# lunarring/latentblending

Hardware: AMD Instinct MI355X
Metric: transition frames/sec, SDXL-Turbo 512x512 4-step 15-branch (higher is better)
Workload: dtype f16; 1 GPU; SDXL-Turbo 512x512, num_inference_steps=4, nmb_max_branches=15 (17 frames/transition), fp16, fixed_seeds=[420,421], anchors not recycled; frontier_width=16, hipgraphs=True, parallelism=single GPU

## Files before the change

### include/lb_hip.h

```cpp
#ifndef LB_HIP_H
#define LB_HIP_H

#include <stdint.h>

#ifdef __cplusplus
extern "C" {
#endif

typedef uint16_t lb_half;

int lb_version(void);
const char* lb_last_error_string(void);
int lb_device_info(int device, int* cu_count, long* lds_per_cu, char* arch, int arch_len);

int lb_slerp_pairs_f16(const void* const* p0, const void* const* p1, void* const* out,
                       const double* fracts, int npairs, long n, void* stream);
int lb_slerp_pairs_f32(const void* const* p0, const void* const* p1, void* const* out,
                       const double* fracts, int npairs, long n, void* stream);
int lb_slerp_pairs_f64(const void* const* p0, const void* const* p1, void* const* out,
                       const double* fracts, int npairs, long n, void* stream);
int lb_slerp_batched_f16(const void* p0, const void* p1, void* out, const double* fracts_dev,
                         long npairs, long n, void* stream);
int lb_slerp_strided_f16(const void* p0, long stride0, const void* p1, long stride1, void* out,
                         const double* fracts_dev, long npairs, long n, void* stream);
// ... 12 lines not shown

enum {
    LB_GEMM_OUT_F32 = 1,
    LB_GEMM_RES_F32 = 2,
    LB_GEMM_GEGLU = 4,
    LB_GEMM_TRANS_OUT = 8,
    LB_GEMM_SILU = 16,
    LB_GEMM_RELU = 32,
    LB_GEMM_QUICK_GELU = 128,
    LB_GEMM_GELU = 256,
    LB_GEMM_CH_STATS = 512,
    LB_GEMM_HALO_RAGGED = 1024,
    LB_GEMM_HALO_KSPLIT = 4096,
    LB_GEMM_C64 = 2048,
    LB_GEMM_GN_A = 8192,
    LB_GEMM_LN_A = 64
};

typedef struct LbGemmParams {
    const lb_half* A;
    const lb_half* W;
    void* C;
    const float* bias;
    const void* residual;
    const lb_half* rowvec;
    float* partial;
    int M, N, K;
    int lda, ldw, ldc, ldr, ld_rowvec, rows_per_batch;
    float alpha;
    int flags;
// ... 14 lines not shown
} LbGemmParams;

int lb_gemm_f16(const LbGemmParams* params, void* stream);
long lb_gemm_workspace_bytes(int M, int N);
void lb_gemm_set_tuning(int tile, int splitk);
void lb_gemm_set_pp_auto(int on);
void lb_gemm_pp_set_group(int gm);
void lb_gemm_set_depth(int depth);
int lb_gemm_plan(const LbGemmParams* p, int* tile, int* splitk, long* blocks);
int lb_conv3x3_halo_f16(const LbGemmParams* params, void* stream);
int lb_conv3x3_narrow_f16(const LbGemmParams* params, void* stream);
void lb_conv_halo_set_persistent(int on);
void lb_conv_halo_plan(const LbGemmParams* params, int* kind, int* tile_w, long* items, long* grid);
#include "lb_hip_ksplit.h"
#include "lb_hip_gn_a.h"
int lb_gemm_ch_stat_rows(const LbGemmParams* params);
int lb_upconv2x_halo_f16(const LbGemmParams* params, void* stream);
void lb_gemm_set_halo(int mode);
void lb_gemm_set_wide_store(int on);
void lb_gemm_set_t192_waves8(int on);
void lb_gemm_set_kgroups(int on);
void lb_gemm_set_lean_epilogue(int on);
void lb_gemm_set_variant(int variant, int stages);

void lb_groupnorm_set_l3_chunk(long bytes);
int lb_groupnorm_from_stats(const void* x, void* y, const float* gamma, const float* beta, const float* ch_stats,
                            void* workspace, int B, int HW, int C, int ldx, int ldy, int groups, float eps, int silu,
                            int x_is_f32, int stat_rows_per_sample, void* stream);
long lb_groupnorm_workspace_bytes(int B, int groups);
int lb_groupnorm_nhwc(const void* x, void* y, const float* gamma, const float* beta, void* workspace,
// ... 81 lines not shown
```

### latentblending_amd/csrc/conv3_narrow.hip

```cpp
#include "lb_common.h"
#include "lb_gemm.h"

typedef __attribute__((address_space(1))) const void* gptr_t;
typedef __attribute__((address_space(3))) void* lptr_t;

#define NARROW_T 16
#define NARROW_HW (NARROW_T + 2)
#define NARROW_HR (NARROW_HW * NARROW_HW)
#define NARROW_HRG ((NARROW_HR + 7) / 8)
#define NARROW_LDS (NARROW_HRG * 8 * 64)

template <bool GNA>
__global__ void __launch_bounds__(256, 2) conv3x3_narrow_kernel(const LbGemmParams p) {
    __shared__ __attribute__((aligned(16))) f16 halo[NARROW_LDS];
    const int tid = threadIdx.x, lane = tid & 63, wave = tid >> 6;
    const int g = lane >> 4, l16 = lane & 15;
    const int tiles_x = p.Win / NARROW_T, tiles_y = p.Hin / NARROW_T;
    int tile = blockIdx.x;
    const int x0 = (tile % tiles_x) * NARROW_T;
    tile /= tiles_x;
    const int y0 = (tile % tiles_y) * NARROW_T;
    const int b = tile / tiles_y;
    const lb_half* zero = reinterpret_cast<const lb_half*>(p.zero_page);
    const int nchunks = p.Cin / 64;
// ... 84 lines not shown
            float o[4];
#pragma unroll
            for (int r = 0; r < 4; ++r) o[r] = acc[i][r] * p.alpha + bias[r];
            if (p.flags & LB_GEMM_OUT_F32)
                *reinterpret_cast<f32x4*>((float*)p.C + m * p.ldc + n) = (f32x4){o[0], o[1], o[2], o[3]};
            else
                *reinterpret_cast<f16x4*>((f16*)p.C + m * p.ldc + n) = (f16x4){(f16)o[0], (f16)o[1], (f16)o[2], (f16)o[3]};
        }
    }
}

int lb_conv3x3_narrow_eligible(const LbGemmParams& p) {
    if (!p.conv || p.KH != 3 || p.KW != 3 || p.stride != 1 || p.pad != 1 || p.ups || p.scatter) return 0;
    if (p.Hout != p.Hin || p.Wout != p.Win || p.Cin % 64 != 0 || p.K != 9 * p.Cin) return 0;
    if (p.N > 16 || p.N % 4 != 0 || p.zero_page == nullptr) return 0;
    if (p.flags & ~(LB_GEMM_OUT_F32 | LB_GEMM_HALO_KSPLIT | LB_GEMM_GN_A)) return 0;
    if (p.residual != nullptr || p.rowvec != nullptr) return 0;
    if (p.Win % NARROW_T != 0 || p.Hin % NARROW_T != 0 || p.M % (p.Hin * p.Win) != 0) return 0;
    if ((long)p.M * p.ldx >= (1l << 34)) return 0;
    return 1;
}

static long narrow_tiles(const LbGemmParams& p) {
    return (long)(p.M / (p.Hin * p.Win)) * (p.Hin / NARROW_T) * (p.Win / NARROW_T);
}

int lb_conv3x3_narrow_check(const LbGemmParams& p) {
    LB_REQUIRE(narrow_tiles(p) < (1l << 31), "conv3x3 narrow: too many tiles for one launch");
    LB_REQUIRE(!(p.flags & LB_GEMM_GN_A) || (p.gn_table != nullptr && (reinterpret_cast<uintptr_t>(p.gn_table) & 15) == 0),
               "conv3x3 narrow: LB_GEMM_GN_A needs gn_table = the 16-byte aligned [B][Cin] float2 table of lb_groupnorm_affine_from_stats");
    return 0;
// ... 21 lines not shown
```

### latentblending_amd/csrc/gemm.hip

```cpp
#include "lb_common.h"
#include "lb_gemm.h"

#define BK 64

template <int N> struct Int { static constexpr int value = N; };

template <int BM, int BN, bool CONV, bool GEGLU, int D>
__global__ void __launch_bounds__(256) gemm_f16_kernel(const LbGemmParams p) {
    constexpr int AI = BM * 8 / 256;
    constexpr int WI = BN * 8 / 256;
    constexpr int TM = BM / 32;
    constexpr int TN = BN / 32;
    __shared__ __attribute__((aligned(16))) f16 lds[2 * (BM + BN) * BK];
    f16* const As = lds;
    f16* const Ws = lds + 2 * BM * BK;

    const int tid = threadIdx.x;
    const int lane = tid & 63, wave = tid >> 6;
    const int wave_m = wave >> 1, wave_n = wave & 1;
    const int g = lane >> 4, l16 = lane & 15;

    const int n_blocks = GEGLU ? (p.N / 2 + BN / 2 - 1) / (BN / 2) : (p.N + BN - 1) / BN;
    int bid = blockIdx.x;
    {
// ... 263 lines not shown
int lb_upconv_halo_launch(LbGemmParams p, hipStream_t stream);
int lb_conv3_c64_check(const LbGemmParams& p);
int lb_conv3_c64_launch(LbGemmParams p, hipStream_t stream);
void lb_conv3_c64_grid(const LbGemmParams& p, long& items, long& grid);
#define LB_HALO_MIN_BLOCKS 96
static int g_halo = 1;
extern "C" void lb_gemm_set_halo(int mode) { g_halo = mode; }
static bool use_halo(const LbGemmParams& p) {
    if (g_halo == 0 || g_force_tile || !lb_conv3x3_halo_eligible(p)) return false;
    return g_halo == 2 || lb_conv3x3_halo_blocks(p) >= LB_HALO_MIN_BLOCKS;
}

int lb_gemm_pp_eligible(const LbGemmParams& p);
int lb_gemm_launch_pp(const LbGemmParams& p, dim3 grid, hipStream_t stream);
int lb_gemm_launch_glds(const LbGemmParams& p, int tile, int stages, dim3 grid, hipStream_t stream);
void lb_gemm_glds_init();
static int g_variant = 1, g_stages = 0;
extern "C" void lb_gemm_set_variant(int variant, int stages) {
    g_variant = variant < 0 ? 1 : variant;
    g_stages = variant < 0 ? 0 : stages;
    if (variant == 1) lb_gemm_glds_init();
}

int g_lb_wide_store = 1;
extern "C" void lb_gemm_set_wide_store(int on) { g_lb_wide_store = on; }
int g_lb_lean_epilogue = 1;
extern "C" void lb_gemm_set_lean_epilogue(int on) { g_lb_lean_epilogue = on; }

extern "C" long lb_gemm_workspace_bytes(int M, int N) {
    return (long)16 * M * N * (long)sizeof(float);
}

template <int BM, int BN>
static void launch_depth(const LbGemmParams& p, int depth, dim3 grid, hipStream_t stream) {
    switch (depth) {
        case 1: launch_variant<BM, BN, 1>(p, grid, stream); break;
        case 2: launch_variant<BM, BN, 2>(p, grid, stream); break;
        case 3: launch_variant<BM, BN, 3>(p, grid, stream); break;
        default: launch_variant<BM, BN, 4>(p, grid, stream); break;
    }
}

static int default_depth(const LbGemmParams& p, int tile) {
    if (tile == 1) return p.conv ? 1 : 3;
    if (tile == 2) return 3;
    return 4;
}

static int gemm_launch_impl(LbGemmParams p, int tile, int depth, int variant, int stages, dim3 grid,
                            hipStream_t stream) {
    if (tile == 9) {
        lb_gemm_launch_pp(p, grid, stream);
    } else if (variant == 1 && p.zero_page != nullptr) {
        lb_gemm_launch_glds(p, tile, stages, grid, stream);
    } else {
        if (depth <= 0) depth = default_depth(p, tile);
        if (tile == 1) launch_depth<128, 128>(p, depth, grid, stream);
        else if (tile == 2) launch_depth<128, 64>(p, depth, grid, stream);
        else launch_depth<64, 64>(p, depth, grid, stream);
    }
    int rc = lb_check_launch("lb_gemm_f16");
    if (rc) return rc;
    if (p.splitk > 1) {
        const long quads = (long)p.M * (p.N / 4);
        long gsz = (quads + 255) / 256;
// ... 71 lines not shown
        if (splitk > k_tiles) splitk = k_tiles;
        if (splitk < 1) splitk = 1;
        if (tile == 9 && !g_force_splitk) splitk = 1;
        if (tile >= 4 && tile != 11 && !g_force_splitk) splitk = 1;
    }
    if (!g_force_tile && g_kgroups && tile == 3 && splitk == 1 && !p.conv && g_variant == 1 && p.zero_page != nullptr && nblk <= 200 &&
        (p.K + BK - 1) / BK >= 8)
        tile = 11;
    tile_out = tile;
    splitk_out = splitk;
    nblk_out = nblk;
}

extern "C" int lb_gemm_plan(const LbGemmParams* pp, int* tile, int* splitk, long* blocks) {
    LB_REQUIRE(pp != nullptr && pp->M > 0 && pp->N > 0 && pp->K > 0, "lb_gemm_plan: empty problem");
    int t = 0, sk = 1;
    long nb = 0;
    if (pp->flags & LB_GEMM_C64) {
        if (const int rc = lb_conv3_c64_check(*pp)) return rc;
        long items = 0;
        t = 12;
        lb_conv3_c64_grid(*pp, items, nb);
    }
    else if (g_halo != 0 && !g_force_tile && lb_conv3x3_narrow_eligible(*pp)) { t = 8; nb = (long)pp->M / 256; }
    else if (use_halo(*pp)) { t = 6; nb = lb_conv3x3_halo_blocks(*pp); }
    else if (pp->flags & LB_GEMM_HALO_KSPLIT) {
        LbGemmParams q = *pp;
        q.flags &= ~LB_GEMM_HALO_KSPLIT;
        q.partial = nullptr;
        gemm_plan(q, t, sk, nb);
// ... 30 lines not shown
            k = 8;
            f = lb_conv_halo_gn_a_mode() != 0;
        } else if (use_halo(p) && lb_conv3x3_halo_gn_a_able(p)) {
            k = 3;
            f = lb_conv3x3_halo_gn_a_policy(p);
        }
    }
    if (fuse) *fuse = f;
    if (kind) *kind = k;
}

extern "C" int lb_gemm_f16(const LbGemmParams* pp, void* stream) {
    LbGemmParams p = *pp;
    const bool geglu = (p.flags & LB_GEMM_GEGLU) != 0;
    LB_REQUIRE(p.M > 0 && p.N > 0 && p.K > 0, "lb_gemm_f16: empty problem");
    LB_REQUIRE(p.K % 8 == 0 && p.ldw % 8 == 0, "lb_gemm_f16: K and ldw must be multiples of 8");
    LB_REQUIRE(p.N % 4 == 0 && (geglu ? p.N % 8 == 0 : true), "lb_gemm_f16: N must be a multiple of 4");
    LB_REQUIRE(p.ldc % 4 == 0 || (p.flags & LB_GEMM_TRANS_OUT), "lb_gemm_f16: ldc must be a multiple of 4");
    if (p.conv) {
        LB_REQUIRE(p.Cin % 8 == 0 && p.ldx % 8 == 0, "lb_gemm_f16: conv Cin/ldx must be multiples of 8");
        LB_REQUIRE(p.K == p.KH * p.KW * p.Cin, "lb_gemm_f16: conv K != KH*KW*Cin");
        LB_REQUIRE(p.M % (p.Hout * p.Wout) == 0, "lb_gemm_f16: conv M must be B*Hout*Wout");
        if (p.scatter)
            LB_REQUIRE(p.KH == 2 && p.KW == 2 && p.stride == 1 && p.ups == 0 && p.Hout == p.Hin && p.Wout == p.Win &&
                           !(p.flags & (LB_GEMM_TRANS_OUT | LB_GEMM_GEGLU)) && p.residual == nullptr,
                       "lb_gemm_f16: sub-pixel conv needs KH=KW=2, stride 1, Hout=Hin, no residual");
    } else {
        LB_REQUIRE(p.lda % 8 == 0, "lb_gemm_f16: lda must be a multiple of 8");
    }
    if (p.flags & LB_GEMM_LN_A) {
// ... 21 lines not shown
        if (const int rc = lb_conv3x3_halo_check(p)) return rc;
        LB_DISPATCH("lb_conv3x3_halo_f16", lb_conv3x3_halo_launch(p, s));
    }
    LB_REQUIRE(!(p.flags & LB_GEMM_GN_A), "lb_gemm_f16: LB_GEMM_GN_A is implemented by the whole-tile 3x3 halo conv and the narrow-N conv only "
                                          "(ask lb_conv_halo_gn_a_plan before flagging a conv)");
    if (p.flags & LB_GEMM_HALO_KSPLIT) {
        p.flags &= ~LB_GEMM_HALO_KSPLIT;
        p.partial = nullptr;
    }
    LB_REQUIRE(!(p.flags & LB_GEMM_CH_STATS), "lb_gemm_f16: LB_GEMM_CH_STATS is implemented by the halo-tile conv kernels only "
                                              "(check lb_gemm_plan == 6 / lb_conv_halo_plan before asking for it)");
    int tile = 0, splitk = 1;
    long nblk = 0;
    gemm_plan(p, tile, splitk, nblk);
    p.splitk = splitk;
    const int depth = g_depth, variant = g_variant;
    int stages = g_stages;
    if (variant == 1) {
        lb_gemm_glds_init();
        if (stages == 0)
            stages = (tile == 3 || tile == 4 || tile == 7 || tile == 10 || tile == 11) ? 3 : 2;
    }
    const dim3 grid((unsigned)nblk, 1, (unsigned)splitk);
    LB_DISPATCH("lb_gemm_f16", gemm_launch_impl(p, tile, depth, variant, stages, grid, s));
}
```

### latentblending_amd/csrc/gemm_glds.hip

```cpp
#include <type_traits>
#include "lb_common.h"
#include "lb_gemm.h"

#define BK 64
#ifndef LB_GLDS_LEAN
#define LB_GLDS_LEAN 1
#endif
#ifndef LB_ABLATE
#define LB_ABLATE 0
#endif
#ifndef LB_BURST
#define LB_BURST 0
#endif
typedef __attribute__((address_space(1))) const void* gptr_t;
typedef __attribute__((address_space(3))) void* lptr_t;

template <int N> __device__ __forceinline__ void wait_vm_barrier() {
    asm volatile("s_waitcnt vmcnt(%0)\n\ts_barrier" ::"n"(N) : "memory");
}

typedef _Float16 lb_h2 __attribute__((ext_vector_type(2)));
template <int TM>
__device__ __forceinline__ void ln_accumulate(const f16x8 (&af)[TM], float (&sum)[TM], float (&sq)[TM]) {
    const lb_h2 one2 = {(f16)1.f, (f16)1.f};
#pragma unroll
    for (int i = 0; i < TM; ++i)
#pragma unroll
        for (int e = 0; e < 4; ++e) {
            const lb_h2 x = {af[i][2 * e], af[i][2 * e + 1]};
            sum[i] = __builtin_amdgcn_fdot2(x, one2, sum[i], false);
            sq[i] = __builtin_amdgcn_fdot2(x, x, sq[i], false);
        }
}

template <int BM, int BN, bool CONV, bool GEGLU, int S, int WMW, int LNA = 0, int KG = 1>
__global__ void __launch_bounds__(WMW * 128 * KG) gemm_f16_glds_kernel(const LbGemmParams p) {
    static_assert(KG == 1 || !CONV, "K-groups: plain / GEGLU GEMMs only");
    constexpr int NT = WMW * 128;
    constexpr int RPI = NT / 8;
    constexpr int AI = BM * 8 / NT;
    constexpr int WI = (BN * 8 + NT - 1) / NT;
    constexpr int NL = AI + WI;
    constexpr int WROWS = BM / WMW;
    constexpr int WPAD = WI * RPI;
    static_assert(BM * 8 % NT == 0, "A tile rows must be a whole number of staging rounds");
    constexpr int TM = WROWS / 16, TN = BN / 32;
    constexpr int STAGE = (BM + WPAD) * BK;
    extern __shared__ __attribute__((aligned(16))) f16 lds_all[];

    const int kgrp = KG > 1 ? __builtin_amdgcn_readfirstlane((int)threadIdx.x / NT) : 0;
    const int tid = KG > 1 ? (int)threadIdx.x - kgrp * NT : (int)threadIdx.x;
    f16* const lds = lds_all + kgrp * (S * STAGE);
// ... 293 lines not shown
                for (int j = 0; j < TN; ++j) {
                    const f32x4 o = *reinterpret_cast<const f32x4*>(theirs + ((i * TN + j) * 64 + lane) * 4);
#pragma unroll
                    for (int r = 0; r < 4; ++r) acc[i][j][r] += o[r];
                }
            if (LNA) {
#pragma unroll
                for (int i = 0; i < TM; ++i) {
                    ln_sum[i] += theirs[TM * TN * 256 + (2 * i) * 64 + lane];
                    ln_sq[i] += theirs[TM * TN * 256 + (2 * i + 1) * 64 + lane];
                }
            }
        }
    }

    if (p.splitk > 1) {
        float* slab = p.partial + (long)blockIdx.z * p.M * p.N;
#pragma unroll
        for (int i = 0; i < TM; ++i) {
            const int m = m0 + wave_m * WROWS + i * 16 + l16;
            if (m >= p.M) continue;
#pragma unroll
            for (int j = 0; j < TN; ++j) {
                const int n = n0 + wave_n * (BN / 2) + j * 16 + 4 * g;
                if (n < p.N) *reinterpret_cast<f32x4*>(slab + (long)m * p.N + n) = acc[i][j];
            }
        }
        return;
    }
    if (LNA) {
// ... 39 lines not shown
    return BM + WI * RPI;
}

template <int BM, int BN, int S, int WMW, int KG>
static int launch_glds_kgroups(const LbGemmParams& p, dim3 grid, hipStream_t stream) {
    const size_t smem = (size_t)KG * S * glds_stage_rows<BM, BN, WMW>() * BK * sizeof(f16);
    const bool geglu = (p.flags & LB_GEMM_GEGLU) != 0, lna = (p.flags & LB_GEMM_LN_A) != 0;
    const dim3 block(WMW * 128 * KG);
    if (geglu && lna) hipLaunchKernelGGL((gemm_f16_glds_kernel<BM, BN, false, true, S, WMW, 1, KG>), grid, block, smem, stream, p);
    else if (geglu) hipLaunchKernelGGL((gemm_f16_glds_kernel<BM, BN, false, true, S, WMW, 0, KG>), grid, block, smem, stream, p);
    else if (lna) hipLaunchKernelGGL((gemm_f16_glds_kernel<BM, BN, false, false, S, WMW, 1, KG>), grid, block, smem, stream, p);
    else hipLaunchKernelGGL((gemm_f16_glds_kernel<BM, BN, false, false, S, WMW, 0, KG>), grid, block, smem, stream, p);
    return 0;
}

template <int BM, int BN, int S, int WMW = 2>
static int launch_glds_variant(const LbGemmParams& p, dim3 grid, hipStream_t stream) {
    const size_t smem = (size_t)S * glds_stage_rows<BM, BN, WMW>() * BK * sizeof(f16);
    const bool geglu = (p.flags & LB_GEMM_GEGLU) != 0;
    const dim3 block(WMW * 128);
    const bool lna = (p.flags & LB_GEMM_LN_A) != 0;
    if (p.conv) hipLaunchKernelGGL((gemm_f16_glds_kernel<BM, BN, true, false, S, WMW>), grid, block, smem, stream, p);
    else if (geglu && lna) hipLaunchKernelGGL((gemm_f16_glds_kernel<BM, BN, false, true, S, WMW, 1>), grid, block, smem, stream, p);
    else if (geglu) hipLaunchKernelGGL((gemm_f16_glds_kernel<BM, BN, false, true, S, WMW>), grid, block, smem, stream, p);
    else if (lna) hipLaunchKernelGGL((gemm_f16_glds_kernel<BM, BN, false, false, S, WMW, 1>), grid, block, smem, stream, p);
    else hipLaunchKernelGGL((gemm_f16_glds_kernel<BM, BN, false, false, S, WMW>), grid, block, smem, stream, p);
    return 0;
}

template <int BM, int BN, int S, int WMW = 2>
static void allow_lds() {
    const int smem = S * glds_stage_rows<BM, BN, WMW>() * BK * (int)sizeof(f16);
    hipFuncSetAttribute(reinterpret_cast<const void*>(gemm_f16_glds_kernel<BM, BN, true, false, S, WMW>),
                        hipFuncAttributeMaxDynamicSharedMemorySize, smem);
    hipFuncSetAttribute(reinterpret_cast<const void*>(gemm_f16_glds_kernel<BM, BN, false, true, S, WMW>),
                        hipFuncAttributeMaxDynamicSharedMemorySize, smem);
// ... 13 lines not shown
    allow_lds<128, 64, 2, 2>(); allow_lds<128, 64, 3>(); allow_lds<128, 64, 4>();
    allow_lds<64, 64, 2>(); allow_lds<64, 64, 3, 2>(); allow_lds<64, 64, 4>();
    allow_lds<256, 128, 2, 4>(); allow_lds<256, 128, 3, 4>();
    allow_lds<256, 256, 2, 4>();
    allow_lds<192, 128, 3, 3>();
    allow_lds<192, 128, 3, 4>();
    {
        const int smem = 2 * 3 * glds_stage_rows<64, 64, 2>() * BK * (int)sizeof(f16);
        hipFuncSetAttribute(reinterpret_cast<const void*>(gemm_f16_glds_kernel<64, 64, false, true, 3, 2, 1, 2>), hipFuncAttributeMaxDynamicSharedMemorySize, smem);
        hipFuncSetAttribute(reinterpret_cast<const void*>(gemm_f16_glds_kernel<64, 64, false, true, 3, 2, 0, 2>), hipFuncAttributeMaxDynamicSharedMemorySize, smem);
        hipFuncSetAttribute(reinterpret_cast<const void*>(gemm_f16_glds_kernel<64, 64, false, false, 3, 2, 1, 2>), hipFuncAttributeMaxDynamicSharedMemorySize, smem);
        hipFuncSetAttribute(reinterpret_cast<const void*>(gemm_f16_glds_kernel<64, 64, false, false, 3, 2, 0, 2>), hipFuncAttributeMaxDynamicSharedMemorySize, smem);
    }
}

int lb_gemm_launch_glds(const LbGemmParams& p, int tile, int stages, dim3 grid, hipStream_t stream) {
    if (tile == 7) return launch_glds_variant<192, 128, 3, 3>(p, grid, stream);
    if (tile == 10) return launch_glds_variant<192, 128, 3, 4>(p, grid, stream);
    if (tile == 11) {
        if (p.conv) return launch_glds_variant<64, 64, 3, 2>(p, grid, stream);
        return launch_glds_kgroups<64, 64, 3, 2, 2>(p, grid, stream);
    }
    if (tile == 5) return launch_glds_variant<256, 256, 2, 4>(p, grid, stream);
    if (tile == 4) {
        if (stages == 3) return launch_glds_variant<256, 128, 3, 4>(p, grid, stream);
        return launch_glds_variant<256, 128, 2, 4>(p, grid, stream);
    }
    if (tile == 1) {
        if (stages == 2) return launch_glds_variant<128, 128, 2, 2>(p, grid, stream);
        if (stages == 4) return launch_glds_variant<128, 128, 4>(p, grid, stream);
// ... 12 lines not shown
```

### latentblending_amd/csrc/lb_gemm.h

```cpp
#pragma once
#include "lb_common.h"
#include "../../include/lb_hip.h"

typedef _Float16 lb_h2x __attribute__((ext_vector_type(2)));

__device__ __forceinline__ void lb_gemm_store4(const LbGemmParams& p, int m, int n, int bidx, f32x4 v) {
    float o[4];
#pragma unroll
    for (int r = 0; r < 4; ++r) o[r] = v[r] * p.alpha;
    if (p.bias) {
        const f32x4 b = *reinterpret_cast<const f32x4*>(p.bias + n);
#pragma unroll
        for (int r = 0; r < 4; ++r) o[r] += b[r];
    }
    if (p.rowvec) {
        const f16x4 t = *reinterpret_cast<const f16x4*>(
            reinterpret_cast<const f16*>(p.rowvec) + (long)bidx * p.ld_rowvec + n);
#pragma unroll
        for (int r = 0; r < 4; ++r) o[r] += (float)t[r];
    }
    if (p.residual) {
        if (p.flags & LB_GEMM_RES_F32) {
            const f32x4 q = *reinterpret_cast<const f32x4*>((const float*)p.residual + (long)m * p.ldr + n);
#pragma unroll
            for (int r = 0; r < 4; ++r) o[r] += q[r];
        } else {
            const f16x4 q = *reinterpret_cast<const f16x4*>((const f16*)p.residual + (long)m * p.ldr + n);
#pragma unroll
            for (int r = 0; r < 4; ++r) o[r] += (float)q[r];
        }
    }
    if (p.flags & LB_GEMM_SILU) {
#pragma unroll
        for (int r = 0; r < 4; ++r) o[r] = lb_silu(o[r]);
    }
    if (p.flags & LB_GEMM_RELU) {
#pragma unroll
        for (int r = 0; r < 4; ++r) o[r] = fmaxf(o[r], 0.f);
    }
    if (p.flags & (LB_GEMM_QUICK_GELU | LB_GEMM_GELU)) {
#pragma unroll
        for (int r = 0; r < 4; ++r) o[r] = (p.flags & LB_GEMM_GELU) ? lb_gelu_erf(o[r]) : lb_quick_gelu(o[r]);
    }
    long crow = m;
// ... 438 lines not shown
```

### latentblending_amd/hip/lib.py

```python
from __future__ import annotations

import ctypes as C
import os

import torch

_HERE = os.path.dirname(os.path.abspath(__file__))
LIB_PATH = os.environ.get("LB_HIP_LIBRARY") or os.path.join(_HERE, "liblbhip.so")

c_void_pp = C.POINTER(C.c_void_p)


class LbGemmParams(C.Structure):
    _fields_ = [
        ("A", C.c_void_p), ("W", C.c_void_p), ("C", C.c_void_p), ("bias", C.c_void_p),
        ("residual", C.c_void_p), ("rowvec", C.c_void_p), ("partial", C.c_void_p),
        ("M", C.c_int), ("N", C.c_int), ("K", C.c_int),
        ("lda", C.c_int), ("ldw", C.c_int), ("ldc", C.c_int), ("ldr", C.c_int),
        ("ld_rowvec", C.c_int), ("rows_per_batch", C.c_int),
        ("alpha", C.c_float), ("flags", C.c_int),
        ("conv", C.c_int), ("Hin", C.c_int), ("Win", C.c_int), ("Cin", C.c_int),
        ("Hout", C.c_int), ("Wout", C.c_int), ("KH", C.c_int), ("KW", C.c_int),
        ("stride", C.c_int), ("pad", C.c_int), ("ups", C.c_int), ("ldx", C.c_int),
        ("splitk", C.c_int), ("zero_page", C.c_void_p),
# ... 5 lines not shown

class LbAttnParams(C.Structure):
    _fields_ = [
        ("Q", C.c_void_p), ("K", C.c_void_p), ("V", C.c_void_p), ("O", C.c_void_p),
        ("B", C.c_int), ("H", C.c_int), ("Sq", C.c_int), ("Skv", C.c_int), ("Skv_valid", C.c_int),
        ("ldq", C.c_int), ("ldk", C.c_int), ("ldv", C.c_int), ("ldo", C.c_int),
        ("scale", C.c_float), ("causal", C.c_int), ("zero_page", C.c_void_p), ("reserved_", C.c_int),
    ]


GEMM_OUT_F32, GEMM_RES_F32, GEMM_GEGLU, GEMM_TRANS_OUT, GEMM_SILU, GEMM_RELU, GEMM_LN_A = 1, 2, 4, 8, 16, 32, 64
GEMM_QUICK_GELU, GEMM_GELU, GEMM_CH_STATS = 128, 256, 512
GEMM_HALO_RAGGED = 1024
GEMM_HALO_KSPLIT = 4096
GEMM_GN_A = 8192
GEMM_C64 = 2048

_vp, _i, _l, _f, _d = C.c_void_p, C.c_int, C.c_long, C.c_float, C.c_double

SIGNATURES = {
    "lb_version": (_i, []),
    "lb_last_error_string": (C.c_char_p, []),
    "lb_device_info": (_i, [_i, C.POINTER(_i), C.POINTER(_l), C.c_char_p, _i]),
    "lb_slerp_pairs_f16": (_i, [c_void_pp, c_void_pp, c_void_pp, C.POINTER(_d), _i, _l, _vp]),
    "lb_slerp_pairs_f32": (_i, [c_void_pp, c_void_pp, c_void_pp, C.POINTER(_d), _i, _l, _vp]),
    "lb_slerp_pairs_f64": (_i, [c_void_pp, c_void_pp, c_void_pp, C.POINTER(_d), _i, _l, _vp]),
    "lb_slerp_batched_f16": (_i, [_vp, _vp, _vp, _vp, _l, _l, _vp]),
    "lb_slerp_strided_f16": (_i, [_vp, _l, _vp, _l, _vp, _vp, _l, _l, _vp]),
    "lb_lerp_f16": (_i, [_vp, _vp, _vp, _l, _d, _vp]),
    "lb_lerp_f32": (_i, [_vp, _vp, _vp, _l, _d, _vp]),
# ... 71 lines not shown
    "lb_conv_halo_set_study": (None, [_i]),
}

HOST_SIGNATURES = {
    "lb_conv_halo_ksplit_plan": (None, [C.POINTER(LbGemmParams), C.POINTER(C.c_long), C.POINTER(C.c_long), C.POINTER(C.c_int)]),
    "lb_conv_halo_ksplit_workspace_bytes": (_l, [C.POINTER(LbGemmParams)]),
    "lb_conv_halo_set_ksplit": (None, [_i, _i]),
}

GN_A_SIGNATURES = {
    "lb_groupnorm_affine_from_stats": (_i, [_vp, _vp, _vp, _vp, _i, _i, _i, _i, _f, _i, _vp]),
    "lb_conv_halo_gn_a_plan": (None, [C.POINTER(LbGemmParams), C.POINTER(C.c_int), C.POINTER(C.c_int)]),
    "lb_conv_halo_set_gn_a": (None, [_i, _i]),
}

_NO_CHECK = {"lb_version", "lb_last_error_string", "lb_gemm_workspace_bytes", "lb_jpeg_coefficient_count", "lb_jpeg_workspace_bytes",
             "lb_groupnorm_workspace_bytes", "lb_groupnorm_set_l3_chunk", "lb_conv_halo_set_persistent", "lb_conv_halo_plan","lb_gemm_ch_stat_rows", "lb_conv_halo_set_study", "lb_gemm_set_tuning", "lb_gemm_set_depth", "lb_gemm_set_variant", "lb_gemm_set_wide_store", "lb_gemm_set_lean_epilogue", "lb_gemm_set_t192_waves8", "lb_gemm_set_kgroups", "lb_gemm_pp_set_group", "lb_gemm_set_pp_auto", "lb_gemm_set_policy", "lb_gemm_set_halo", "lb_attn_set_tuning", "lb_layernorm_set_form", "lb_groupnorm_set_fused", "lb_groupnorm_plan", "lb_slerp_set_study", "lb_program_create",
             "lb_program_destroy", "lb_program_recording", "lb_program_num_ops", "lb_program_op_name"}


def _load():
    if not os.path.isfile(LIB_PATH):
        raise ImportError(
            f"latentblending_amd: {LIB_PATH} is missing. Build it with "
            "`python -c 'import __graft_entry__ as g; g.build()'` (hipcc, gfx950). "
            "There is no CPU fallback for the kernel path.")
    return C.CDLL(LIB_PATH, mode=C.RTLD_GLOBAL)


_lib = _load()
# ... 13 lines not shown
    checked.__name__ = name
    return checked


api = _Api()
for _name, (_res, _args) in SIGNATURES.items():
    _fn = getattr(_lib, _name)
    _fn.restype = _res
    _fn.argtypes = _args
    setattr(api, _name, _fn if _name in _NO_CHECK else _wrap(_name, _fn))
for _name, (_res, _args) in HOST_SIGNATURES.items():
    _fn = getattr(_lib, _name)
    _fn.restype = _res
    _fn.argtypes = _args
    setattr(api, _name, _fn)
for _name, (_res, _args) in GN_A_SIGNATURES.items():
    _fn = getattr(_lib, _name)
    _fn.restype = _res
    _fn.argtypes = _args
    setattr(api, _name, _wrap(_name, _fn) if _res is _i else _fn)
for _name, (_res, _args) in STUDY_SIGNATURES.items():
    _fn = getattr(_lib, _name, None)
    if _fn is not None:
        _fn.restype = _res
        _fn.argtypes = _args
        setattr(api, _name, _fn)

if os.environ.get("LB_GEMM_WIDE_STORE"):
    api.lb_gemm_set_wide_store(int(os.environ["LB_GEMM_WIDE_STORE"]))
if os.environ.get("LB_GEMM_LEAN_EPILOGUE"):
# ... 4 lines not shown
```

### latentblending_amd/native/runtime.py

```python
from __future__ import annotations

import contextlib
import ctypes as C
from typing import Dict, List, Optional, Tuple

import torch

from ..hip import lib
from ..hip.lib import api, LbGemmParams, LbAttnParams
from .geometry import use_ragged_halo

F16, F32 = torch.float16, torch.float32


class Arena:
    def __init__(self, device):
        self.device = device
        self.free: Dict[int, List[torch.Tensor]] = {}
        self.all: List[torch.Tensor] = []
        self.bytes_allocated = 0

    @staticmethod
    def _cls(nbytes: int) -> int:
        return max(512, (nbytes + 511) // 512 * 512)
# ... 99 lines not shown
class Emitter:

    def __init__(self, arena: Arena):
        self.arena = arena
        self.device = arena.device
        self.ws_gemm: Optional[torch.Tensor] = None
        self.ws_gn: Optional[torch.Tensor] = None
        self.gemm_log: List[dict] = []
        self.attn_log: List[dict] = []
        self.norm_log: List[dict] = []
        self._retired: List[torch.Tensor] = []
        self.zero_page = torch.zeros(64, dtype=torch.uint8, device=self.device)
        self.ragged_halo = False
        self.halo_ksplit = True
        self.ws_ksplit: Optional[torch.Tensor] = None
        self.gn_a = True

    def _ragged_flag(self, p: LbGemmParams) -> int:
        if not self.ragged_halo or not p.conv or p.KH != 3 or p.KW != 3 or p.stride != 1 or p.scatter or p.ups or p.N <= 16:
            return 0
        kind, tw = C.c_int(), C.c_int()
        flags = p.flags
        p.flags = flags & ~lib.GEMM_HALO_RAGGED
        api.lb_conv_halo_plan(C.byref(p), C.byref(kind), None, None, None)
        plain = kind.value
        p.flags = flags | lib.GEMM_HALO_RAGGED
        api.lb_conv_halo_plan(C.byref(p), C.byref(kind), C.byref(tw), None, None)
        p.flags = flags
        return lib.GEMM_HALO_RAGGED if use_ragged_halo(True, plain, kind.value, p.Hin, p.Win, tw.value) else 0

    def _gemm_ws(self, M: int, N: int) -> Optional[torch.Tensor]:
        if ((M + 63) // 64) * ((N + 63) // 64) > 640:
            return None
        need = api.lb_gemm_workspace_bytes(M, N) // 4
        if self.ws_gemm is None or self.ws_gemm.numel() < need:
            if self.ws_gemm is not None:
                self._retired.append(self.ws_gemm)
            self.ws_gemm = torch.empty(max(need, 1 << 22), dtype=F32, device=self.device)
        return self.ws_gemm

    _KSPLIT_COUNTER_BYTES = 1 << 20

    def _halo_ksplit(self, p: LbGemmParams) -> bool:
        if not self.halo_ksplit or not p.conv or p.KH != 3 or p.KW != 3 or p.stride != 1 or p.scatter or p.ups:
            return False
        tile, sk, nb = C.c_int(), C.c_int(), C.c_long()
        api.lb_gemm_plan(C.byref(p), C.byref(tile), C.byref(sk), C.byref(nb))
        if tile.value != 6:
            return False
        flags = p.flags
        p.flags = flags | lib.GEMM_HALO_KSPLIT
        units, grid, split = C.c_long(), C.c_long(), C.c_int()
        api.lb_conv_halo_ksplit_plan(C.byref(p), C.byref(units), C.byref(grid), C.byref(split))
        need = int(api.lb_conv_halo_ksplit_workspace_bytes(C.byref(p)))
# ... 95 lines not shown
            p.lda = lda if lda is not None else K
        p.ldc = ldc if ldc is not None else (M if flags & lib.GEMM_TRANS_OUT else n_out)
        p.ldr = ldr if ldr is not None else n_out
        if rowvec is not None:
            p.ld_rowvec, p.rows_per_batch = ld_rowvec if ld_rowvec is not None else N, rows_per_batch
        p.alpha, p.flags = alpha, flags
        p.zero_page = self.zero_page.data_ptr()
        if ln is not None:
            p.flags |= lib.GEMM_LN_A
            p.ln_colsum, p.ln_eps = ln[0].data_ptr(), float(ln[1])
        if ch_stats is not None:
            assert conv is not None and ch_stats.dtype == F32
            p.flags |= lib.GEMM_CH_STATS
            p.ch_stats, p.ch_stats_rows = ch_stats.data_ptr(), ch_stats.shape[1]
        if splitk and not (flags & lib.GEMM_GEGLU) and ln is None:
            p.partial = _p(self._gemm_ws(M, N))
        if self.ragged_halo:
            p.flags |= self._ragged_flag(p)
        if conv is not None:
            self._halo_ksplit(p)
        return p

    def plan(self, M: int, N: int, K: int, flags: int = 0) -> Tuple[int, int]:
        p = LbGemmParams()
        p.M, p.N, p.K, p.flags = M, N, K, flags
        p.zero_page = self.zero_page.data_ptr()
        if not (flags & lib.GEMM_GEGLU):
            p.partial = _p(self._gemm_ws(M, N))
        t, sk, nb = C.c_int(), C.c_int(), C.c_long()
        api.lb_gemm_plan(C.byref(p), C.byref(t), C.byref(sk), C.byref(nb))
        return t.value, sk.value

    def halo_stat_rows(self, B: int, H: int, W: int, cin: int, cout: int, ks: int = 3) -> int:
        p = LbGemmParams()
        p.conv, p.M, p.N, p.K = 1, B * H * W, cout, ks * ks * cin
# ... 58 lines not shown
```

Before: 128.7 frames/s.

## Fuse split-K reduction into GEMM launch via last-block ticket counter

Adds an in-launch split-K path to the glds GEMM. Each K-slice block writes its fp32 partial tile to a per-tile slab and bumps an atomic counter, and the last block to arrive sums all slabs and runs the full epilogue (bias, rowvec, residual, activation). This removes the separate reduction kernel launch and the extra full M×N partial-buffer round trip that split-K needed before. In exchange it adds atomics, a dedicated zero-initialised workspace whose counters must reset each launch, and serialised reduction work in the last block of each tile.

Measured after the change: 128.7 frames/s. Within noise of the previous version (-0.0%).

```diff
diff --git a/include/lb_hip.h b/include/lb_hip.h
--- a/include/lb_hip.h
+++ b/include/lb_hip.h
@@ -50,6 +50,7 @@
     LB_GEMM_HALO_KSPLIT = 4096,
     LB_GEMM_C64 = 2048,
     LB_GEMM_GN_A = 8192,
+    LB_GEMM_SPLITK_INLAUNCH = 16384,
     LB_GEMM_LN_A = 64
 };
 
@@ -94,6 +95,7 @@
 void lb_conv_halo_plan(const LbGemmParams* params, int* kind, int* tile_w, long* items, long* grid);
 #include "lb_hip_ksplit.h"
 #include "lb_hip_gn_a.h"
+#include "lb_hip_splitk.h"
 int lb_gemm_ch_stat_rows(const LbGemmParams* params);
 int lb_upconv2x_halo_f16(const LbGemmParams* params, void* stream);
 void lb_gemm_set_halo(int mode);
diff --git a/include/lb_hip_splitk.h b/include/lb_hip_splitk.h
--- /dev/null
+++ b/include/lb_hip_splitk.h
@@ -0,0 +1,11 @@
+#ifndef LB_HIP_SPLITK_H
+#define LB_HIP_SPLITK_H
+#ifdef __cplusplus
+extern "C" {
+#endif
+long lb_gemm_splitk_inlaunch_workspace_bytes(int M, int N);
+void lb_gemm_set_splitk_inlaunch(int mode);
+#ifdef __cplusplus
+}
+#endif
+#endif
diff --git a/latentblending_amd/csrc/conv3_narrow.hip b/latentblending_amd/csrc/conv3_narrow.hip
--- a/latentblending_amd/csrc/conv3_narrow.hip
+++ b/latentblending_amd/csrc/conv3_narrow.hip
@@ -122,7 +122,7 @@
     if (!p.conv || p.KH != 3 || p.KW != 3 || p.stride != 1 || p.pad != 1 || p.ups || p.scatter) return 0;
     if (p.Hout != p.Hin || p.Wout != p.Win || p.Cin % 64 != 0 || p.K != 9 * p.Cin) return 0;
     if (p.N > 16 || p.N % 4 != 0 || p.zero_page == nullptr) return 0;
-    if (p.flags & ~(LB_GEMM_OUT_F32 | LB_GEMM_HALO_KSPLIT | LB_GEMM_GN_A)) return 0;
+    if (p.flags & ~(LB_GEMM_OUT_F32 | LB_GEMM_HALO_KSPLIT | LB_GEMM_GN_A | LB_GEMM_SPLITK_INLAUNCH)) return 0;
     if (p.residual != nullptr || p.rowvec != nullptr) return 0;
     if (p.Win % NARROW_T != 0 || p.Hin % NARROW_T != 0 || p.M % (p.Hin * p.Win) != 0) return 0;
     if ((long)p.M * p.ldx >= (1l << 34)) return 0;
diff --git a/latentblending_amd/csrc/gemm.hip b/latentblending_amd/csrc/gemm.hip
--- a/latentblending_amd/csrc/gemm.hip
+++ b/latentblending_amd/csrc/gemm.hip
@@ -301,6 +301,8 @@
 int lb_gemm_pp_eligible(const LbGemmParams& p);
 int lb_gemm_launch_pp(const LbGemmParams& p, dim3 grid, hipStream_t stream);
 int lb_gemm_launch_glds(const LbGemmParams& p, int tile, int stages, dim3 grid, hipStream_t stream);
+int lb_gemm_glds_splitk_inlaunch_able(const LbGemmParams& p, int tile, int stages);
+int lb_gemm_launch_glds_splitk_inlaunch(const LbGemmParams& p, int tile, dim3 grid, hipStream_t stream);
 void lb_gemm_glds_init();
 static int g_variant = 1, g_stages = 0;
 extern "C" void lb_gemm_set_variant(int variant, int stages) {
@@ -317,6 +319,16 @@
 extern "C" long lb_gemm_workspace_bytes(int M, int N) {
     return (long)16 * M * N * (long)sizeof(float);
 }
+
+static long splitk_inlaunch_counter_bytes(int M, int N) {
+    return (((long)((M + 63) / 64) * ((N + 63) / 64) * 4 + 255) / 256) * 256;
+}
+extern "C" long lb_gemm_splitk_inlaunch_workspace_bytes(int M, int N) {
+    if (M <= 0 || N <= 0) return 0;
+    return splitk_inlaunch_counter_bytes(M, N) + (long)16 * ((M + 127) / 128 * 128) * ((N + 63) / 64 * 64) * (long)sizeof(float);
+}
+static int g_splitk_inlaunch = 1;
+extern "C" void lb_gemm_set_splitk_inlaunch(int mode) { g_splitk_inlaunch = mode; }
 
 template <int BM, int BN>
 static void launch_depth(const LbGemmParams& p, int depth, dim3 grid, hipStream_t stream) {
@@ -334,8 +346,15 @@
     return 4;
 }
 
-static int gemm_launch_impl(LbGemmParams p, int tile, int depth, int variant, int stages, dim3 grid,
+static int gemm_launch_impl(LbGemmParams p, int tile, int depth, int variant, int stages, int inlaunch, dim3 grid,
                             hipStream_t stream) {
+    if ((p.flags & LB_GEMM_SPLITK_INLAUNCH) && p.partial != nullptr) {
+        if (inlaunch && tile != 9 && variant == 1 && p.zero_page != nullptr && p.splitk <= 16 && lb_gemm_glds_splitk_inlaunch_able(p, tile, stages)) {
+            lb_gemm_launch_glds_splitk_inlaunch(p, tile, grid, stream);
+            return lb_check_launch("lb_gemm_f16");
+        }
+        p.partial = reinterpret_cast<float*>(reinterpret_cast<char*>(p.partial) + splitk_inlaunch_counter_bytes(p.M, p.N));
+    }
     if (tile == 9) {
         lb_gemm_launch_pp(p, grid, stream);
     } else if (variant == 1 && p.zero_page != nullptr) {
@@ -437,6 +456,8 @@
 
 extern "C" int lb_gemm_plan(const LbGemmParams* pp, int* tile, int* splitk, long* blocks) {
     LB_REQUIRE(pp != nullptr && pp->M > 0 && pp->N > 0 && pp->K > 0, "lb_gemm_plan: empty problem");
+    LB_REQUIRE(!((pp->flags & LB_GEMM_HALO_KSPLIT) && (pp->flags & LB_GEMM_SPLITK_INLAUNCH)),
+               "lb_gemm_plan: LB_GEMM_HALO_KSPLIT and LB_GEMM_SPLITK_INLAUNCH each give `partial` a meaning of their own: one per launch");
     int t = 0, sk = 1;
     long nb = 0;
     if (pp->flags & LB_GEMM_C64) {
@@ -497,6 +518,8 @@
     LbGemmParams p = *pp;
     const bool geglu = (p.flags & LB_GEMM_GEGLU) != 0;
     LB_REQUIRE(p.M > 0 && p.N > 0 && p.K > 0, "lb_gemm_f16: empty problem");
+    LB_REQUIRE(!((p.flags & LB_GEMM_HALO_KSPLIT) && (p.flags & LB_GEMM_SPLITK_INLAUNCH)),
+               "lb_gemm_f16: LB_GEMM_HALO_KSPLIT and LB_GEMM_SPLITK_INLAUNCH each give `partial` a meaning of their own: one per launch");
     LB_REQUIRE(p.K % 8 == 0 && p.ldw % 8 == 0, "lb_gemm_f16: K and ldw must be multiples of 8");
     LB_REQUIRE(p.N % 4 == 0 && (geglu ? p.N % 8 == 0 : true), "lb_gemm_f16: N must be a multiple of 4");
     LB_REQUIRE(p.ldc % 4 == 0 || (p.flags & LB_GEMM_TRANS_OUT), "lb_gemm_f16: ldc must be a multiple of 4");
@@ -548,7 +571,7 @@
     long nblk = 0;
     gemm_plan(p, tile, splitk, nblk);
     p.splitk = splitk;
-    const int depth = g_depth, variant = g_variant;
+    const int depth = g_depth, variant = g_variant, inlaunch = g_splitk_inlaunch;
     int stages = g_stages;
     if (variant == 1) {
         lb_gemm_glds_init();
@@ -556,5 +579,5 @@
             stages = (tile == 3 || tile == 4 || tile == 7 || tile == 10 || tile == 11) ? 3 : 2;
     }
     const dim3 grid((unsigned)nblk, 1, (unsigned)splitk);
-    LB_DISPATCH("lb_gemm_f16", gemm_launch_impl(p, tile, depth, variant, stages, grid, s));
-}
+    LB_DISPATCH("lb_gemm_f16", gemm_launch_impl(p, tile, depth, variant, stages, inlaunch, grid, s));
+}
diff --git a/latentblending_amd/csrc/gemm_glds.hip b/latentblending_amd/csrc/gemm_glds.hip
--- a/latentblending_amd/csrc/gemm_glds.hip
+++ b/latentblending_amd/csrc/gemm_glds.hip
@@ -33,9 +33,10 @@
         }
 }
 
-template <int BM, int BN, bool CONV, bool GEGLU, int S, int WMW, int LNA = 0, int KG = 1>
+template <int BM, int BN, bool CONV, bool GEGLU, int S, int WMW, int LNA = 0, int KG = 1, int SKI = 0>
 __global__ void __launch_bounds__(WMW * 128 * KG) gemm_f16_glds_kernel(const LbGemmParams p) {
     static_assert(KG == 1 || !CONV, "K-groups: plain / GEGLU GEMMs only");
+    static_assert(!SKI || (KG == 1 && !GEGLU && !LNA && WMW == 2), "in-launch split-K sum: 4-wave plain / conv tiles only");
     constexpr int NT = WMW * 128;
     constexpr int RPI = NT / 8;
     constexpr int AI = BM * 8 / NT;
@@ -359,6 +360,87 @@
         }
     }
 
+    if constexpr (SKI != 0) {
+        if (p.splitk > 1) {
+            typedef unsigned u32x4 __attribute__((ext_vector_type(4)));
+            constexpr int SLAB = BM * BN * 4;
+            const long ctr_bytes = (((long)((p.M + 63) / 64) * ((p.N + 63) / 64) * 4 + 255) / 256) * 256;
+            int* const counter = reinterpret_cast<int*>(p.partial) + bid;
+            char* const slabs = reinterpret_cast<char*>(p.partial) + ctr_bytes + (long)bid * p.splitk * SLAB;
+            const __amdgpu_buffer_rsrc_t srs = __builtin_amdgcn_make_buffer_rsrc(slabs, 0, p.splitk * SLAB, 0x00020000);
+            const int voff = tid * 16;
+#pragma unroll
+            for (int i = 0; i < TM; ++i)
+#pragma unroll
+                for (int j = 0; j < TN; ++j)
+                    __builtin_amdgcn_raw_buffer_store_b128(__builtin_bit_cast(u32x4, acc[i][j]), srs, voff,
+                                                           (int)blockIdx.z * SLAB + (i * TN + j) * 4096, 16);
+            volatile int* const flag = reinterpret_cast<volatile int*>(lds_all);
+            asm volatile("s_waitcnt vmcnt(0)" ::: "memory");
+            __syncthreads();
+            if (tid == 0) {
+                const int ticket = __hip_atomic_fetch_add(counter, 1, __ATOMIC_RELAXED, __HIP_MEMORY_SCOPE_AGENT);
+                const bool last_one = ticket == p.splitk - 1;
+                if (last_one) __hip_atomic_store(counter, 0, __ATOMIC_RELAXED, __HIP_MEMORY_SCOPE_AGENT);
+                *flag = last_one ? 1 : 0;
+            }
+            __syncthreads();
+            if (__builtin_amdgcn_readfirstlane(*flag) == 0) return;
+            LbStore4Operands eo[TM][TN];
+            f32x4 eb[TN];
+#pragma unroll
+            for (int j = 0; j < TN; ++j) {
+                const int n = n0 + wave_n * (BN / 2) + j * 16 + 4 * g;
+                eb[j] = p.bias ? *reinterpret_cast<const f32x4*>(p.bias + (n < p.N ? n : 0)) : (f32x4){0.f, 0.f, 0.f, 0.f};
+            }
+#pragma unroll
+            for (int i = 0; i < TM; ++i) {
+                const int m = m0 + wave_m * WROWS + i * 16 + l16;
+                const int mc = m < p.M ? m : p.M - 1;
+#pragma unroll
+                for (int j = 0; j < TN; ++j) {
+                    const int n = n0 + wave_n * (BN / 2) + j * 16 + 4 * g;
+                    eo[i][j] = lb_gemm_store4_load(p, mc, n < p.N ? n : 0, p.rowvec ? mc / p.rows_per_batch : 0);
+                }
+            }
+#pragma unroll
+            for (int i = 0; i < TM; ++i)
+#pragma unroll
+                for (int j = 0; j < TN; ++j) acc[i][j] = (f32x4){0.f, 0.f, 0.f, 0.f};
+            constexpr int ZB = 16 / (TM * TN);
+            for (int z0 = 0; z0 < p.splitk; z0 += ZB) {
+                f32x4 part[ZB][TM][TN];
+#pragma unroll
+                for (int zz = 0; zz < ZB; ++zz) {
+                    const int z = z0 + zz < p.splitk ? z0 + zz : p.splitk - 1;
+#pragma unroll
+                    for (int i = 0; i < TM; ++i)
+#pragma unroll
+                        for (int j = 0; j < TN; ++j)
+                            part[zz][i][j] = __builtin_bit_cast(f32x4, __builtin_amdgcn_raw_buffer_load_b128(srs, voff, z * SLAB + (i * TN + j) * 4096, 16));
+                }
+#pragma unroll
+                for (int zz = 0; zz < ZB; ++zz) {
+                    if (z0 + zz >= p.splitk) break;
+#pragma unroll
+                    for (int i = 0; i < TM; ++i)
+#pragma unroll
+                        for (int j = 0; j < TN; ++j) acc[i][j] += part[zz][i][j];
+                }
+            }
+#pragma unroll
+            for (int i = 0; i < TM; ++i) {
+                const int m = m0 + wave_m * WROWS + i * 16 + l16;
+                if (m >= p.M) continue;
+#pragma unroll
+                for (int j = 0; j < TN; ++j) {
+                    const int n = n0 + wave_n * (BN / 2) + j * 16 + 4 * g;
+                    if (n < p.N) lb_gemm_store4_finish(p, m, n, eo[i][j], eb[j], acc[i][j]);
+                }
+            }
+            return;
+        }
+    }
     if (p.splitk > 1) {
         float* slab = p.partial + (long)blockIdx.z * p.M * p.N;
 #pragma unroll
@@ -428,12 +510,17 @@
     return 0;
 }
 
-template <int BM, int BN, int S, int WMW = 2>
+template <int BM, int BN, int S, int WMW = 2, int SKI = 0>
 static int launch_glds_variant(const LbGemmParams& p, dim3 grid, hipStream_t stream) {
     const size_t smem = (size_t)S * glds_stage_rows<BM, BN, WMW>() * BK * sizeof(f16);
     const bool geglu = (p.flags & LB_GEMM_GEGLU) != 0;
     const dim3 block(WMW * 128);
     const bool lna = (p.flags & LB_GEMM_LN_A) != 0;
+    if constexpr (SKI != 0) {
+        if (p.conv) hipLaunchKernelGGL((gemm_f16_glds_kernel<BM, BN, true, false, S, WMW, 0, 1, 1>), grid, block, smem, stream, p);
+        else hipLaunchKernelGGL((gemm_f16_glds_kernel<BM, BN, false, false, S, WMW, 0, 1, 1>), grid, block, smem, stream, p);
+        return 0;
+    }
     if (p.conv) hipLaunchKernelGGL((gemm_f16_glds_kernel<BM, BN, true, false, S, WMW>), grid, block, smem, stream, p);
     else if (geglu && lna) hipLaunchKernelGGL((gemm_f16_glds_kernel<BM, BN, false, true, S, WMW, 1>), grid, block, smem, stream, p);
     else if (geglu) hipLaunchKernelGGL((gemm_f16_glds_kernel<BM, BN, false, true, S, WMW>), grid, block, smem, stream, p);
@@ -477,6 +564,14 @@
     }
 }
 
+int lb_gemm_glds_splitk_inlaunch_able(const LbGemmParams& p, int tile, int stages) {
+    return p.splitk > 1 && !(p.flags & (LB_GEMM_GEGLU | LB_GEMM_LN_A)) && ((tile == 3 && stages == 3) || (tile == 2 && stages == 2));
+}
+int lb_gemm_launch_glds_splitk_inlaunch(const LbGemmParams& p, int tile, dim3 grid, hipStream_t stream) {
+    if (tile == 2) return launch_glds_variant<128, 64, 2, 2, 1>(p, grid, stream);
+    return launch_glds_variant<64, 64, 3, 2, 1>(p, grid, stream);
+}
+
 int lb_gemm_launch_glds(const LbGemmParams& p, int tile, int stages, dim3 grid, hipStream_t stream) {
     if (tile == 7) return launch_glds_variant<192, 128, 3, 3>(p, grid, stream);
     if (tile == 10) return launch_glds_variant<192, 128, 3, 4>(p, grid, stream);
diff --git a/latentblending_amd/csrc/lb_gemm.h b/latentblending_amd/csrc/lb_gemm.h
--- a/latentblending_amd/csrc/lb_gemm.h
+++ b/latentblending_amd/csrc/lb_gemm.h
@@ -28,6 +28,78 @@
             const f16x4 q = *reinterpret_cast<const f16x4*>((const f16*)p.residual + (long)m * p.ldr + n);
 #pragma unroll
             for (int r = 0; r < 4; ++r) o[r] += (float)q[r];
+        }
+    }
+    if (p.flags & LB_GEMM_SILU) {
+#pragma unroll
+        for (int r = 0; r < 4; ++r) o[r] = lb_silu(o[r]);
+    }
+    if (p.flags & LB_GEMM_RELU) {
+#pragma unroll
+        for (int r = 0; r < 4; ++r) o[r] = fmaxf(o[r], 0.f);
+    }
+    if (p.flags & (LB_GEMM_QUICK_GELU | LB_GEMM_GELU)) {
+#pragma unroll
+        for (int r = 0; r < 4; ++r) o[r] = (p.flags & LB_GEMM_GELU) ? lb_gelu_erf(o[r]) : lb_quick_gelu(o[r]);
+    }
+    long crow = m;
+    if (p.scatter) {
+        const int hw = p.Hout * p.Wout;
+        const int b = m / hw, rem = m - b * hw;
+        const int y = rem / p.Wout, x = rem - y * p.Wout;
+        crow = ((long)b * 2 * p.Hout + 2 * y + p.sc_py) * (2 * p.Wout) + 2 * x + p.sc_px;
+    }
+    if (p.flags & LB_GEMM_TRANS_OUT) {
+        f16* c = (f16*)p.C;
+#pragma unroll
+        for (int r = 0; r < 4; ++r) c[(long)(n + r) * p.ldc + m] = (f16)o[r];
+    } else if (p.flags & LB_GEMM_OUT_F32) {
+        *reinterpret_cast<f32x4*>((float*)p.C + crow * p.ldc + n) = (f32x4){o[0], o[1], o[2], o[3]};
+    } else {
+        *reinterpret_cast<f16x4*>((f16*)p.C + crow * p.ldc + n) =
+            (f16x4){(f16)o[0], (f16)o[1], (f16)o[2], (f16)o[3]};
+    }
+}
+
+struct LbStore4Operands { f32x4 q; f16x4 t; };
+__device__ __forceinline__ LbStore4Operands lb_gemm_store4_load(const LbGemmParams& p, int m, int n, int bidx) {
+    LbStore4Operands e;
+    e.q = (f32x4){0.f, 0.f, 0.f, 0.f};
+    e.t = (f16x4){0, 0, 0, 0};
+    if (p.rowvec) e.t = *reinterpret_cast<const f16x4*>(reinterpret_cast<const f16*>(p.rowvec) + (long)bidx * p.ld_rowvec + n);
+    if (p.residual) {
+        if (p.flags & LB_GEMM_RES_F32) {
+            e.q = *reinterpret_cast<const f32x4*>((const float*)p.residual + (long)m * p.ldr + n);
+        } else {
+            typedef float lb_f2 __attribute__((ext_vector_type(2)));
+            const lb_f2 h = __builtin_bit_cast(lb_f2, *reinterpret_cast<const f16x4*>((const f16*)p.residual + (long)m * p.ldr + n));
+            e.q[0] = h[0];
+            e.q[1] = h[1];
+        }
+    }
+    return e;
+}
+__device__ __forceinline__ void lb_gemm_store4_finish(const LbGemmParams& p, int m, int n, const LbStore4Operands& e, f32x4 b, f32x4 v) {
+    float o[4];
+#pragma unroll
+    for (int r = 0; r < 4; ++r) o[r] = v[r] * p.alpha;
+    if (p.bias) {
+#pragma unroll
+        for (int r = 0; r < 4; ++r) o[r] += b[r];
+    }
+    if (p.rowvec) {
+#pragma unroll
+        for (int r = 0; r < 4; ++r) o[r] += (float)e.t[r];
+    }
+    if (p.residual) {
+        if (p.flags & LB_GEMM_RES_F32) {
+#pragma unroll
+            for (int r = 0; r < 4; ++r) o[r] += e.q[r];
+        } else {
+            typedef float lb_f2 __attribute__((ext_vector_type(2)));
+            const f16x4 q16 = __builtin_bit_cast(f16x4, (lb_f2){e.q[0], e.q[1]});
+#pragma unroll
+            for (int r = 0; r < 4; ++r) o[r] += (float)q16[r];
         }
     }
     if (p.flags & LB_GEMM_SILU) {
diff --git a/latentblending_amd/hip/lib.py b/latentblending_amd/hip/lib.py
--- a/latentblending_amd/hip/lib.py
+++ b/latentblending_amd/hip/lib.py
@@ -43,6 +43,7 @@
 GEMM_HALO_RAGGED = 1024
 GEMM_HALO_KSPLIT = 4096
 GEMM_GN_A = 8192
+GEMM_SPLITK_INLAUNCH = 16384
 GEMM_C64 = 2048
 
 _vp, _i, _l, _f, _d = C.c_void_p, C.c_int, C.c_long, C.c_float, C.c_double
@@ -144,6 +145,11 @@
     "lb_conv_halo_set_gn_a": (None, [_i, _i]),
 }
 
+SPLITK_SIGNATURES = {
+    "lb_gemm_splitk_inlaunch_workspace_bytes": (_l, [_i, _i]),
+    "lb_gemm_set_splitk_inlaunch": (None, [_i]),
+}
+
 _NO_CHECK = {"lb_version", "lb_last_error_string", "lb_gemm_workspace_bytes", "lb_jpeg_coefficient_count", "lb_jpeg_workspace_bytes",
              "lb_groupnorm_workspace_bytes", "lb_groupnorm_set_l3_chunk", "lb_conv_halo_set_persistent", "lb_conv_halo_plan","lb_gemm_ch_stat_rows", "lb_conv_halo_set_study", "lb_gemm_set_tuning", "lb_gemm_set_depth", "lb_gemm_set_variant", "lb_gemm_set_wide_store", "lb_gemm_set_lean_epilogue", "lb_gemm_set_t192_waves8", "lb_gemm_set_kgroups", "lb_gemm_pp_set_group", "lb_gemm_set_pp_auto", "lb_gemm_set_policy", "lb_gemm_set_halo", "lb_attn_set_tuning", "lb_layernorm_set_form", "lb_groupnorm_set_fused", "lb_groupnorm_plan", "lb_slerp_set_study", "lb_program_create",
              "lb_program_destroy", "lb_program_recording", "lb_program_num_ops", "lb_program_op_name"}
@@ -187,6 +193,11 @@
     _fn.restype = _res
     _fn.argtypes = _args
     setattr(api, _name, _fn)
+for _name, (_res, _args) in SPLITK_SIGNATURES.items():
+    _fn = getattr(_lib, _name)
+    _fn.restype = _res
+    _fn.argtypes = _args
+    setattr(api, _name, _fn)
 for _name, (_res, _args) in GN_A_SIGNATURES.items():
     _fn = getattr(_lib, _name)
     _fn.restype = _res
diff --git a/latentblending_amd/native/runtime.py b/latentblending_amd/native/runtime.py
--- a/latentblending_amd/native/runtime.py
+++ b/latentblending_amd/native/runtime.py
@@ -137,6 +137,8 @@
         self.ragged_halo = False
         self.halo_ksplit = True
         self.ws_ksplit: Optional[torch.Tensor] = None
+        self.splitk_inlaunch = True
+        self.ws_splitk: Optional[torch.Tensor] = None
         self.gn_a = True
 
     def _ragged_flag(self, p: LbGemmParams) -> int:
@@ -161,6 +163,21 @@
                 self._retired.append(self.ws_gemm)
             self.ws_gemm = torch.empty(max(need, 1 << 22), dtype=F32, device=self.device)
         return self.ws_gemm
+
+    _SPLITK_COUNTER_BYTES = 4096
+
+    def _splitk_ws(self, M: int, N: int) -> Optional[int]:
+        if ((M + 63) // 64) * ((N + 63) // 64) > 640:
+            return None
+        need = int(api.lb_gemm_splitk_inlaunch_workspace_bytes(M, N))
+        counters = (((M + 63) // 64) * ((N + 63) // 64) * 4 + 255) // 256 * 256
+        assert 0 < counters <= self._SPLITK_COUNTER_BYTES and need > counters, (M, N, need, counters)
+        total = self._SPLITK_COUNTER_BYTES + need - counters
+        if self.ws_splitk is None or self.ws_splitk.numel() * 4 < total:
+            if self.ws_splitk is not None:
+                self._retired.append(self.ws_splitk)
+            self.ws_splitk = torch.zeros(max(total, 1 << 24) // 4, dtype=torch.int32, device=self.device)
+        return self.ws_splitk.data_ptr() + self._SPLITK_COUNTER_BYTES - counters
 
     _KSPLIT_COUNTER_BYTES = 1 << 20
 
@@ -286,11 +303,16 @@
             p.flags |= lib.GEMM_CH_STATS
             p.ch_stats, p.ch_stats_rows = ch_stats.data_ptr(), ch_stats.shape[1]
         if splitk and not (flags & lib.GEMM_GEGLU) and ln is None:
-            p.partial = _p(self._gemm_ws(M, N))
+            if self.splitk_inlaunch:
+                p.partial = self._splitk_ws(M, N)
+                if p.partial:
+                    p.flags |= lib.GEMM_SPLITK_INLAUNCH
+            else:
+                p.partial = _p(self._gemm_ws(M, N))
         if self.ragged_halo:
             p.flags |= self._ragged_flag(p)
-        if conv is not None:
-            self._halo_ksplit(p)
+        if conv is not None and self._halo_ksplit(p):
+            p.flags &= ~lib.GEMM_SPLITK_INLAUNCH
         return p
 
     def plan(self, M: int, N: int, K: int, flags: int = 0) -> Tuple[int, int]:
```
